# zezax/one

Hardware: AMD Instinct MI355X
Metric: GB/s input scanned (and Minput/s) for fixed DFA (higher is better)
Workload: dtype u8; 1 GPU; configs[1]: syn256 DFA (256 states used / 256 classes, REDA fmtDirect4), 1048576 lines x 64 B per GPU, match<styLast,false> -> result+start+end; input=uniformly random bytes, lines_per_gpu=1048576, line_len=64, rotating_input_buffers=6, working_set_bytes=402653184, streams=1, steps_per_call=32

## Files before the change

### one_amd/csrc/k_diag.h

```cpp
#pragma once

__global__ void __launch_bounds__(512)
k_diag_read(const uint4 *__restrict__ p, uint64_t n16, uint32_t *sink) {
  typedef uint32_t v4 __attribute__((ext_vector_type(4)));
  const v4 *q = reinterpret_cast<const v4 *>(p);
  const uint64_t step = uint64_t(gridDim.x) * 512;
  uint64_t i = uint64_t(blockIdx.x) * 512 + threadIdx.x;
  v4 acc = {0, 0, 0, 0};
  for (; i + 7 * step < n16; i += 8 * step) {
    v4 v[8];
#pragma unroll
    for (int k = 0; k < 8; ++k) v[k] = __builtin_nontemporal_load(q + i + k * step);
#pragma unroll
    for (int k = 0; k < 8; ++k) acc ^= v[k];
  }
  for (; i < n16; i += step) acc ^= q[i];
  uint32_t a = acc.x ^ acc.y ^ acc.z ^ acc.w;
  for (int o = 32; o; o >>= 1) a ^= __shfl_xor(a, o);
  if ((threadIdx.x & 63) == 0 && a == 0x9e3779b9u) atomicAdd(sink, 1u);
}

__global__ void __launch_bounds__(512)
k_diag_lines(const uint8_t *__restrict__ data, uint64_t nLines, int32_t *res, uint64_t *st,
             uint64_t *en, uint32_t *sink) {
  typedef uint32_t v4 __attribute__((ext_vector_type(4)));
  const uint64_t tiles = nLines / 1024;
  const uint64_t G = gridDim.x;
  if (blockIdx.x >= tiles) return;
  const uint64_t Q = (tiles - blockIdx.x + G - 1) / G;
  uint64_t ldT = blockIdx.x, ldQ = 0, t = blockIdx.x;
  v4 acc = {0, 0, 0, 0};
  v4 A[2][4], B[2][4];
  auto issue = [&](v4 (&blk)[2][4]) {
#pragma unroll
    for (int k = 0; k < 4; ++k)
#pragma unroll
      for (int c = 0; c < 2; ++c) {
        const uint64_t ln = ldT * 1024 + uint64_t(c) * 512 + threadIdx.x;
        blk[c][k] = reinterpret_cast<const v4 *>(data + ln * 64)[k];
      }
    if (ldQ + 1 < Q) { ++ldQ; ldT += G; }
  };
  auto walk = [&](const v4 (&blk)[2][4]) {
#pragma unroll
    for (int c = 0; c < 2; ++c) {
      const uint64_t ln = t * 1024 + uint64_t(c) * 512 + threadIdx.x;
      const v4 x = blk[c][0] ^ blk[c][1] ^ blk[c][2] ^ blk[c][3];
      acc ^= x;
      __builtin_nontemporal_store(int32_t(x.x), res + ln);
      __builtin_nontemporal_store(uint64_t(x.z), en + ln);
      __builtin_nontemporal_store(uint64_t(x.y), st + ln);
    }
    t += G;
  };
  issue(A);
  issue(B);
  walk(A);
  issue(A);
  for (uint64_t q = 1; q < Q; q += 2) {
    walk(B);
    if (q + 1 >= Q) break;
    issue(B);
    walk(A);
    issue(A);
  }
  if ((acc.x ^ acc.y ^ acc.z ^ acc.w) == 0x9e3779b9u) atomicAdd(sink, 1u);
}

__global__ void __launch_bounds__(512)
k_diag_long(const uint8_t *__restrict__ data, uint64_t nLines, uint32_t lineBytes, uint32_t *sink) {
  typedef uint32_t v4 __attribute__((ext_vector_type(4)));
  const uint64_t tiles = nLines / 1024;
  const uint32_t R = lineBytes / 128;
  v4 acc = {0, 0, 0, 0};
  for (uint64_t t = blockIdx.x; t < tiles; t += gridDim.x) {
    for (uint32_t r = 0; r < R; ++r) {
      v4 v[2][8];
#pragma unroll
      for (int k = 0; k < 8; ++k)
#pragma unroll
        for (int c = 0; c < 2; ++c) {
          const uint64_t ln = t * 1024 + uint64_t(c) * 512 + threadIdx.x;
          v[c][k] = reinterpret_cast<const v4 *>(data + ln * lineBytes + uint64_t(r) * 128)[k];
        }
#pragma unroll
      for (int c = 0; c < 2; ++c)
#pragma unroll
        for (int k = 0; k < 8; ++k) acc ^= v[c][k];
    }
  }
  if ((acc.x ^ acc.y ^ acc.z ^ acc.w) == 0x9e3779b9u) atomicAdd(sink, 1u);
}

template <int CH>
__global__ void __launch_bounds__(256)
k_diag_l2(const uint16_t *__restrict__ tab, uint32_t rounds, uint32_t *sink) {
  uint32_t idx[CH];
#pragma unroll
  for (int c = 0; c < CH; ++c)
    idx[c] = (blockIdx.x * 256u + threadIdx.x) * 2654435761u + uint32_t(c) * 40503u;
  for (uint32_t r = 0; r < rounds; ++r) {
#pragma unroll
    for (int c = 0; c < CH; ++c) {
      const uint32_t v = tab[idx[c] & 0xfffffu];
      idx[c] = idx[c] * 33u + v + r;
    }
  }
  uint32_t a = 0;
#pragma unroll
  for (int c = 0; c < CH; ++c) a ^= idx[c];
  if (a == 0x9e3779b9u) atomicAdd(sink, 1u);
}
```

### one_amd/csrc/k_stream_multi.h

```cpp
#pragma once

constexpr int kMultiMax = 32;

struct MultiPtrs {
  const uint8_t *data;
  int32_t *result;
  uint64_t *start;
  uint64_t *end;
  uint64_t n;
};

struct MultiIo {
  uint32_t nb;
  uint32_t lineLen;
  uint32_t tileStart[kMultiMax + 1];
  uint32_t ignoreAcceptUpTo;
  MultiPtrs b[kMultiMax];
};

typedef uint32_t u32x4_t __attribute__((ext_vector_type(4)));
__device__ __forceinline__ uint4 ntLoad16(const uint8_t *p) {
  const u32x4_t v = __builtin_nontemporal_load(reinterpret_cast<const u32x4_t *>(p));
  return make_uint4(v.x, v.y, v.z, v.w);
}

template <int MODE, int HALVES, int THREADS, int NT = 2, bool LEAN = false, int GR = 1,
          bool R1 = false>
__global__ void __launch_bounds__(THREADS)
k_stream_multi(DevDfa d, MultiIo m) {
  static_assert(MODE == kSmLastStartEnd || MODE == kSmLastEnd || MODE == kSmFullStart ||
                MODE == kSmFull, "the plain output modes only");
  static_assert(!LEAN || MODE != kSmFull, "styFull without start has no bookkeeping to defer");
  static_assert(GR == 1 || LEAN, "more than two chains per lane: the lean step only");
  static_assert(!R1 || (HALVES == 1 && !LEAN && GR == 1), "R1: the plain 64-byte walk only");
  constexpr uint32_t BLK = 64 * HALVES;
  constexpr int CH = kStreamChains * GR;
  constexpr bool kAcc = MODE == kSmLastStartEnd || MODE == kSmLastEnd;
  constexpr bool kStart = MODE == kSmLastStartEnd || MODE == kSmFullStart;
  constexpr uint32_t LPT = uint32_t(THREADS) * CH;
  __shared__ __align__(16) uint8_t lds[kStreamTabBytes + 1024];
  uint8_t *tab = lds;
  int32_t *ldsRes = reinterpret_cast<int32_t *>(lds + kStreamTabBytes);

  const uint32_t init = d.init, firstAccept = d.firstAccept;
  const uint32_t lineLen = m.lineLen;
  const uint32_t R = R1 ? 1u : lineLen / BLK;
  const uint32_t nTiles = m.tileStart[m.nb];
  const uint32_t G = gridDim.x;
  if (blockIdx.x >= nTiles) return;
  const uint32_t myTiles = (nTiles - blockIdx.x + G - 1) / G;
  const uint64_t Q = uint64_t(myTiles) * R;

  uint32_t ldTile = blockIdx.x, ldR = 0, ldK = 0;
  uint32_t ldLo = 0, ldHi = m.tileStart[1];
  const uint8_t *ldData = m.b[0].data;
  uint64_t ldN = m.b[0].n;
  uint64_t ldQ = 0;
  const uint8_t *ldP[CH];
  auto setLoadTile = [&]() {
    while (ldTile >= ldHi) {
      ++ldK;
      ldLo = ldHi;
      ldHi = m.tileStart[ldK + 1];
      ldData = m.b[ldK].data;
      ldN = m.b[ldK].n;
    }
    const uint64_t first = uint64_t(ldTile - ldLo) * LPT;
#pragma unroll
    for (int c = 0; c < CH; ++c) {
      uint64_t ln = first + uint64_t(c) * THREADS + threadIdx.x;
      if (ln >= ldN) ln = ldN - 1;
      ldP[c] = ldData + ln * lineLen;
    }
  };
  auto issue = [&](BlockRegs<HALVES> (&blk)[CH]) {
    const uint32_t byteOff = ldR * BLK;
#pragma unroll
    for (int k = 0; k < 4 * HALVES; ++k) {
#pragma unroll
      for (int c = 0; c < CH; ++c)
        blk[c].p[k] = (NT & 1)
                          ? ntLoad16(ldP[c] + byteOff + 16 * k)
                          : reinterpret_cast<const uint4 *>(ldP[c] + byteOff)[k];
    }
    if (ldQ + 1 < Q) {
      ++ldQ;
      if (++ldR == R) {
        ldR = 0;
        ldTile += G;
        setLoadTile();
      }
    }
  };

  const uint4 *tsrc = reinterpret_cast<const uint4 *>(d.table);
  const uint32_t n16 = d.tableBytes / 16;
  constexpr uint32_t kStagePieces = (kStreamTabBytes / 16 + THREADS - 1) / THREADS;
  uint4 tv[kStagePieces];
#pragma unroll
  for (uint32_t k = 0; k < kStagePieces; ++k) {
    const uint32_t i = k * THREADS + threadIdx.x;
    tv[k] = i < n16 ? tsrc[i] : make_uint4(0, 0, 0, 0);
  }
  const int32_t myRes = threadIdx.x < d.nStates ? d.result[threadIdx.x] : 0;
  BlockRegs<HALVES> A[CH], B[CH];
  setLoadTile();
  issue(A);
  {
    uint4 *dst = reinterpret_cast<uint4 *>(tab);
#pragma unroll
    for (uint32_t k = 0; k < kStagePieces; ++k) {
      const uint32_t i = k * THREADS + threadIdx.x;
      if (i < kStreamTabBytes / 16) dst[i] = tv[k];
    }
    if (threadIdx.x < 256) ldsRes[threadIdx.x] = myRes;
  }
  asm volatile("" : : "v"(tab) : "memory");
  __syncthreads();

  uint32_t tile = blockIdx.x, r = 0, wkK = 0;
  uint32_t wkLo = 0, wkHi = m.tileStart[1];
  int32_t *oRes = m.b[0].result;
  uint64_t *oStart = m.b[0].start, *oEnd = m.b[0].end;
  uint64_t oN = m.b[0].n;
  const uint8_t *oData = m.b[0].data;
  auto setWalkTile = [&]() {
    while (tile >= wkHi) {
      ++wkK;
      wkLo = wkHi;
      wkHi = m.tileStart[wkK + 1];
      oRes = m.b[wkK].result;
      oStart = m.b[wkK].start;
      oEnd = m.b[wkK].end;
      oN = m.b[wkK].n;
      if (LEAN) oData = m.b[wkK].data;
    }
  };
  setWalkTile();

  uint32_t s[CH], accS[CH], endv[CH], startv[CH];
  uint64_t mA[CH], mB[CH];
  LeanRegs L[GR];
  const uint32_t T8 = firstAccept << 8;

  auto walkLean = [&](const BlockRegs<HALVES> (&blk)[CH]) {
    if (r == 0) {
#pragma unroll
      for (int g = 0; g < GR; ++g) leanBegin(L[g], init);
    }
#pragma unroll
    for (int g = 0; g < GR; ++g) leanPin(L[g]);
    if (GR > 1) leanDrain();
#pragma unroll
    for (int h = 0; h < HALVES; ++h) {
#pragma unroll
      for (int q = 0; q < 4; ++q) {
        uint4 piece[CH];
#pragma unroll
        for (int c = 0; c < CH; ++c) piece[c] = blk[c].p[4 * h + q];
        leanWalk16<kAcc, kStart, GR>(piece, L, T8, init);
      }
    }
    if (GR > 1) leanDrain();
    if (r + 1 == R) {
      const uint32_t lane = threadIdx.x & 63;
      const uint64_t first = uint64_t(tile - wkLo) * LPT;
#pragma unroll
      for (int g = 0; g < GR; ++g) {
        LeanRegs &G = L[g];
        leanEnd(G, T8, init, kAcc, kStart);
        uint64_t ln[2];
        uint4 pa[2], ps[2];
        uint32_t PA[2], PS[2];
#pragma unroll
        for (int c = 0; c < 2; ++c) {
          ln[c] = first + uint64_t(2 * g + c) * THREADS + threadIdx.x;
          const uint64_t lc = ln[c] < oN ? ln[c] : oN - 1;
          const uint8_t *base = oData + lc * lineLen;
          PA[c] = G.recA[c] ? (G.recA[c] >> 8) - 1 : 0;
          PS[c] = G.recS[c] ? (G.recS[c] >> 8) - 1 : 0;
          if (kAcc) pa[c] = *reinterpret_cast<const uint4 *>(base + 16ull * PA[c]);
          if (kStart) ps[c] = *reinterpret_cast<const uint4 *>(base + 16ull * PS[c]);
        }
        int32_t rr[2];
        uint32_t en[2], sv[2];
        if (kAcc) {
          uint32_t s2[2];
          StreamBook b2[2];
          uint64_t u0[2] = {0, 0}, u1[2] = {0, 0};
#pragma unroll
          for (int c = 0; c < 2; ++c) { s2[c] = G.recA[c] & 0xffu; b2[c].acc = 0; b2[c].end = 0; b2[c].start = 0; }
          streamWalk16<kSmLastEnd, 0>(pa, s2, b2, u0, u1, firstAccept, init);
#pragma unroll
          for (int c = 0; c < 2; ++c) {
            uint32_t acc = b2[c].acc, er = b2[c].end;
            if (s2[c] >= firstAccept) { acc = s2[c]; er = 16; }
            const bool hit = G.recA[c] != 0;
            rr[c] = hit ? ldsRes[acc & 0xffu] : 0;
            en[c] = hit ? 16u * PA[c] + er : 0u;
          }
        } else {
#pragma unroll
          for (int c = 0; c < 2; ++c) {
            rr[c] = G.sX[c] >= firstAccept ? ldsRes[G.sX[c] & 0xffu] : 0;
            en[c] = lineLen;
          }
        }
        if (kStart) {
          uint32_t s3[2];
          StreamBook b3[2];
          uint64_t w0[2], w1[2];
#pragma unroll
          for (int c = 0; c < 2; ++c) {
            s3[c] = G.recS[c] & 0xffu;
            b3[c].acc = 0; b3[c].end = 0; b3[c].start = 0;
            w0[c] = __builtin_amdgcn_ballot_w64(s3[c] == init);
            w1[c] = w0[c];
          }
          streamWalk16<kSmFullStart, 0>(ps, s3, b3, w0, w1, firstAccept, init);
#pragma unroll
          for (int c = 0; c < 2; ++c) {
            uint32_t pos = b3[c].start ? b3[c].start - 1 : 0;
            if (((w0[c] >> lane) & 1) && s3[c] != init) pos = 15;
            sv[c] = G.recS[c] ? 16u * PS[c] + pos : 0u;
          }
        }
#pragma unroll
        for (int c = 0; c < 2; ++c) {
          if (ln[c] < oN) {
            __builtin_nontemporal_store(rr[c], oRes + ln[c]);
            if (oEnd) __builtin_nontemporal_store(rr[c] ? uint64_t(en[c]) : uint64_t(0), oEnd + ln[c]);
            if (kStart && oStart)
              __builtin_nontemporal_store(rr[c] ? uint64_t(sv[c]) : uint64_t(0), oStart + ln[c]);
          }
        }
      }
    }
    if (++r == R) {
      r = 0;
      tile += G;
      if (tile < nTiles) setWalkTile();
    }
  };

  auto walkBlock = [&](const BlockRegs<HALVES> (&blk)[CH]) {
    if constexpr (LEAN) {
      walkLean(blk);
    } else {
    if (r == 0) {
#pragma unroll
      for (int c = 0; c < CH; ++c) {
        s[c] = init; accS[c] = 0; endv[c] = 0; startv[c] = 0;
        mA[c] = ~0ull; mB[c] = ~0ull;
      }
    }
#pragma unroll
    for (int h = 0; h < HALVES; ++h) {
      StreamBook b[CH];
#pragma unroll
      for (int c = 0; c < CH; ++c) { b[c].acc = accS[c]; b[c].end = 0; b[c].start = 0; }
      uint4 piece[CH];
#pragma unroll
      for (int c = 0; c < CH; ++c) piece[c] = blk[c].p[4 * h + 0];
      streamWalk16<MODE, 0>(piece, s, b, mA, mB, firstAccept, init);
#pragma unroll
      for (int c = 0; c < CH; ++c) piece[c] = blk[c].p[4 * h + 1];
      streamWalk16<MODE, 1>(piece, s, b, mA, mB, firstAccept, init);
#pragma unroll
      for (int c = 0; c < CH; ++c) piece[c] = blk[c].p[4 * h + 2];
      streamWalk16<MODE, 2>(piece, s, b, mA, mB, firstAccept, init);
#pragma unroll
      for (int c = 0; c < CH; ++c) piece[c] = blk[c].p[4 * h + 3];
      streamWalk16<MODE, 3>(piece, s, b, mA, mB, firstAccept, init);
      const uint32_t off = r * BLK + h * 64;
#pragma unroll
      for (int c = 0; c < CH; ++c) {
        if (kAcc) {
          accS[c] = b[c].acc;
          endv[c] = b[c].end ? off + b[c].end : endv[c];
          if (s[c] >= firstAccept) { accS[c] = s[c]; endv[c] = off + 64; }
          if (endv[c] <= m.ignoreAcceptUpTo) { endv[c] = 0; accS[c] = 0; }
        }
        if (kStart) {
          startv[c] = b[c].start ? off + b[c].start - 1 : startv[c];
          const bool wasInit63 = (mA[c] >> (threadIdx.x & 63)) & 1;
          if (wasInit63 && s[c] != init) startv[c] = off + 63;
        }
      }
    }
    const bool lineEnd = r + 1 == R;
    const uint64_t first = uint64_t(tile - wkLo) * LPT;
#pragma unroll
    for (int c = 0; c < CH; ++c) {
      const uint64_t ln = first + uint64_t(c) * THREADS + threadIdx.x;
      const bool report = lineEnd && ln < oN;
      int32_t rr;
      uint32_t en;
      if (kAcc) {
        rr = ldsRes[accS[c] & 0xffu];
        rr = endv[c] ? rr : 0;
        en = endv[c];
      } else {
        rr = ldsRes[s[c] & 0xffu];
        rr = s[c] >= firstAccept ? rr : 0;
        en = lineLen;
      }
      int32_t *pr = report ? oRes + ln : reinterpret_cast<int32_t *>(d.sink);
      uint64_t *pe = report && oEnd ? oEnd + ln : reinterpret_cast<uint64_t *>(d.sink);
      uint64_t *ps = report && oStart ? oStart + ln : reinterpret_cast<uint64_t *>(d.sink);
      if ((NT & 2) && R == 1) {
        __builtin_nontemporal_store(rr, pr);
        __builtin_nontemporal_store(rr ? uint64_t(en) : uint64_t(0), pe);
        if (kStart) __builtin_nontemporal_store(rr ? uint64_t(startv[c]) : uint64_t(0), ps);
      } else {
        *pr = rr;
        *pe = rr ? uint64_t(en) : 0;
        if (kStart) *ps = rr ? uint64_t(startv[c]) : 0;
      }
    }
    if (++r == R) {
      r = 0;
      tile += G;
      if (tile < nTiles) setWalkTile();
    }
    }
  };

  issue(B);
  walkBlock(A);
  issue(A);
  for (uint64_t q = 1; q < Q; q += 2) {
    walkBlock(B);
    if (q + 1 >= Q) break;
    issue(B);
    walkBlock(A);
    issue(A);
  }
}

inline int multiLabInt(const char *name, int lo, int hi, int dflt) {
  const char *e = getenv(name);
  const int v = e ? atoi(e) : dflt;
  return v < lo || v > hi ? dflt : v;
}

template <int MODE, int NT, bool LEAN>
hipError_t launchStreamMultiN(const DevDfa &d, const MultiIo &m, const LaunchCfg &cfg,
                              hipStream_t stream) {
  static const int wgs = multiLabInt("REDGPU_MULTI_WGS", 1, 2, 2);
  const uint32_t tiles = m.tileStart[m.nb];
  const bool wide = m.lineLen % 128 == 0;
  const uint32_t want = uint32_t(cfg.numCUs) * uint32_t(wide ? 1 : wgs);
  const uint32_t blocks = tiles < want ? tiles : want;
  if constexpr (!LEAN) {
    if (m.lineLen == 64) {
      hipLaunchKernelGGL((k_stream_multi<MODE, 1, kStreamThreads, NT, false, 1, true>), dim3(blocks),
                         dim3(kStreamThreads), 0, stream, d, m);
      return hipGetLastError();
    }
  }
  if (wide)
    hipLaunchKernelGGL((k_stream_multi<MODE, 2, kStreamThreads, NT, LEAN>), dim3(blocks),
                       dim3(kStreamThreads), 0, stream, d, m);
  else
    hipLaunchKernelGGL((k_stream_multi<MODE, 1, kStreamThreads, NT, LEAN>), dim3(blocks),
                       dim3(kStreamThreads), 0, stream, d, m);
  return hipGetLastError();
}

template <int MODE>
hipError_t launchStreamLean4(const DevDfa &d, const MultiIo &m, const LaunchCfg &cfg,
                             hipStream_t stream) {
  MultiIo m4 = m;
  const uint64_t lpt = uint64_t(kStreamThreads) * kStreamChains * 2;
  for (uint32_t k = 0; k < m.nb; ++k)
    m4.tileStart[k + 1] = m4.tileStart[k] + uint32_t((m.b[k].n + lpt - 1) / lpt);
  for (uint32_t k = m.nb; k < uint32_t(kMultiMax); ++k) m4.tileStart[k + 1] = m4.tileStart[m.nb];
  const uint32_t tiles = m4.tileStart[m4.nb];
  const uint32_t blocks = tiles < uint32_t(cfg.numCUs) ? tiles : uint32_t(cfg.numCUs);
  hipLaunchKernelGGL((k_stream_multi<MODE, 1, kStreamThreads, 2, true, 2>), dim3(blocks),
                     dim3(kStreamThreads), 0, stream, d, m4);
  return hipGetLastError();
}

inline bool leanWanted(const MultiIo &m, const LaunchCfg &cfg) {
  static const int lab = multiLabInt("REDGPU_LEAN", 0, 1, 0);
  return (lab || cfg.forceLean) && m.lineLen >= kLeanMinLine && m.lineLen < (1u << 27);
}

template <int MODE>
hipError_t launchStreamMultiT(const DevDfa &d, const MultiIo &m, const LaunchCfg &cfg,
                              hipStream_t stream) {
  if constexpr (MODE != kSmFull) {
    if (leanWanted(m, cfg)) {
      if (cfg.leanChains4) return launchStreamLean4<MODE>(d, m, cfg, stream);
      return launchStreamMultiN<MODE, 2, true>(d, m, cfg, stream);
    }
  }
  if constexpr (MODE == kSmLastStartEnd) {
    static const int nt = multiLabInt("REDGPU_MULTI_NT", 0, 3, 2);
    if (nt == 0) return launchStreamMultiN<MODE, 0, false>(d, m, cfg, stream);
    if (nt == 1) return launchStreamMultiN<MODE, 1, false>(d, m, cfg, stream);
    if (nt == 3) return launchStreamMultiN<MODE, 3, false>(d, m, cfg, stream);
  }
  return launchStreamMultiN<MODE, 2, false>(d, m, cfg, stream);
}
```

### one_amd/csrc/kernels.hip

```cpp
#include "kernels.h"

#include <cstdlib>
#include <type_traits>

#include "../../include/redgpu.h"

#ifndef REDGPU_TU
#define REDGPU_TU 0
#endif
#define REDGPU_TU_STREAM (REDGPU_TU == 0 || REDGPU_TU == 1)
#define REDGPU_TU_RAGGED (REDGPU_TU == 0 || REDGPU_TU == 2)
#define REDGPU_TU_GENERIC (REDGPU_TU == 0 || REDGPU_TU == 3)
#define REDGPU_TU_GREP (REDGPU_TU == 0 || REDGPU_TU == 4)
#define REDGPU_TU_COLLECT_TEXT (REDGPU_TU == 0 || REDGPU_TU == 5)
#define REDGPU_TU_REPLACE_TEXT (REDGPU_TU == 0 || REDGPU_TU == 6)
#define REDGPU_TU_TALLY_TEXT (REDGPU_TU == 0 || REDGPU_TU == 7)

#define REDGPU_KIND_SWITCH(CALL)                                                          \
  switch (d.tableKind) {                                                                  \
  case REDGPU_TAB_LDS_FUSED_U8: return CALL(REDGPU_TAB_LDS_FUSED_U8);                     \
  case REDGPU_TAB_LDS_FUSED_U16: return CALL(REDGPU_TAB_LDS_FUSED_U16);                   \
  case REDGPU_TAB_LDS_CLASS_U16: return CALL(REDGPU_TAB_LDS_CLASS_U16);                   \
  case REDGPU_TAB_GLOBAL_U16: return CALL(REDGPU_TAB_GLOBAL_U16);                         \
  case REDGPU_TAB_HOT_ROWS: return CALL(REDGPU_TAB_HOT_ROWS);                               \
// ... 546 lines not shown
    return e;
  }
  *kernelName = "k_match_all_long";
  const uint64_t c = collectLongChunk(n, chunkBytes, cfg);
  MlBufs b{};
  b.m = (n + c - 1) / c;
  b.chunk = uint32_t(c);
  const uint64_t nb = (b.m + 1023) / 1024;
  auto up16 = [](uint64_t x) { return (x + 15) & ~uint64_t(15); };
  const size_t bytes = up16(b.m * 8) * 2 + up16(nb * 8) * 2 + up16(b.m * 4) * 5 + 64;
  void *scratch = nullptr;
  hipError_t e = raggedScratch(stream, bytes, &scratch);
  if (e != hipSuccess) return e;
  uint8_t *q = static_cast<uint8_t *>(scratch);
  b.esc = reinterpret_cast<uint64_t *>(q); q += up16(b.m * 8);
  b.off = reinterpret_cast<uint64_t *>(q); q += up16(b.m * 8);
  b.blockOff = reinterpret_cast<uint64_t *>(q); q += up16(nb * 8);
  b.blockEsc = reinterpret_cast<uint64_t *>(q); q += up16(nb * 8);
  b.ent = reinterpret_cast<uint32_t *>(q); q += up16(b.m * 4);
  b.exit = reinterpret_cast<uint32_t *>(q); q += up16(b.m * 4);
  b.cnt = reinterpret_cast<uint32_t *>(q); q += up16(b.m * 4);
  b.head = reinterpret_cast<uint32_t *>(q); q += up16(b.m * 4);
  b.work = reinterpret_cast<uint32_t *>(q); q += up16(b.m * 4);
  b.ctl = reinterpret_cast<uint32_t *>(q);
  *ctl = b.ctl;
  const int lead = doLeader && d.leaderLen > 0 ? 1 : 0;
#define ML_CALL(K) launchMatchAllLongK<K>(d, data, n, b, lead, cap, count, result, start, end, cfg, stream)
  REDGPU_KIND_SWITCH(ML_CALL)
#undef ML_CALL
}

template <int KIND>
hipError_t launchReplaceK(const DevDfa &d, const Batch &b, int style, int lead, const uint8_t *repl,
                          uint64_t replLen, uint64_t max, uint64_t *counts, uint64_t *outLens,
                          const uint64_t *outOffsets, uint8_t *out, uint64_t outCap,
                          const LaunchCfg &cfg, hipStream_t stream) {
  constexpr bool kLds = Tab<KIND>::kInLds || KIND == REDGPU_TAB_HOT_ROWS;
  constexpr int kThreads = kLds ? 1024 : 256;
  const size_t ldsBytes = 512 + ldsTableBytes<KIND>(d);
  hipError_t e = setLds(k_replace<KIND, kThreads>, ldsBytes);
  if (e != hipSuccess) return e;
  uint64_t blocks = (b.n + kThreads - 1) / kThreads;
  const uint64_t perCu = kLds ? (ldsBytes <= 80 * 1024 ? 2 : 1) : 8;
  const uint64_t capBlocks = uint64_t(cfg.numCUs) * perCu;
  if (blocks > capBlocks) blocks = capBlocks;
  if (blocks == 0) blocks = 1;
  hipLaunchKernelGGL((k_replace<KIND, kThreads>), dim3(uint32_t(blocks)), dim3(kThreads), ldsBytes,
                     stream, d, b, style, lead, repl, replLen, max, counts, outLens, outOffsets,
                     out, outCap);
  return hipGetLastError();
}

static hipError_t launchReplacePass(const DevDfa &d, const Batch &b, int style, int lead,
                                    const uint8_t *repl, uint64_t replLen, uint64_t max,
                                    uint64_t *counts, uint64_t *outLens,
                                    const uint64_t *outOffsets, uint8_t *out, uint64_t outCap,
                                    const LaunchCfg &cfg, hipStream_t stream) {
#define RP_CALL(K) launchReplaceK<K>(d, b, style, lead, repl, replLen, max, counts, outLens, \
                                     outOffsets, out, outCap, cfg, stream)
  REDGPU_KIND_SWITCH(RP_CALL)
#undef RP_CALL
}

hipError_t launchReplace(const DevDfa &d, const Batch &b, int style, int doLeader,
                         const uint8_t *repl, uint64_t replLen, uint64_t max, uint64_t *counts,
                         uint64_t *outOffsets, uint8_t *out, uint64_t outCap,
                         const LaunchCfg &cfg, hipStream_t stream) {
  if (b.n == 0) return hipSuccess;
  const int lead = doLeader && d.leaderLen > 0;
  const uint64_t nPart = (b.n + 1023) / 1024;
  void *scratch = nullptr;
  hipError_t e = raggedScratch(stream, size_t(b.n + nPart) * 8 + 64, &scratch);
  if (e != hipSuccess) return e;
  uint64_t *lens = static_cast<uint64_t *>(scratch);
  uint64_t *partials = lens + b.n;
  e = launchReplacePass(d, b, style, lead, repl, replLen, max, counts, lens, nullptr, nullptr, 0,
                        cfg, stream);
  if (e != hipSuccess) return e;
  hipLaunchKernelGGL(k_scan_partials, dim3(uint32_t(nPart)), dim3(256), 0, stream, lens, b.n,
                     partials);
  hipLaunchKernelGGL(k_scan_tops, dim3(1), dim3(1024), 0, stream, partials, nPart);
  hipLaunchKernelGGL(k_scan_fill, dim3(uint32_t(nPart)), dim3(256), 0, stream, lens, b.n, partials,
                     outOffsets);
  e = hipGetLastError();
  if (e != hipSuccess || !out) return e;
  return launchReplacePass(d, b, style, lead, repl, replLen, max, counts, lens, outOffsets, out,
                           outCap, cfg, stream);
}

uint64_t splitChunks(uint64_t len) { return (len + kSplitChunk - 1) / kSplitChunk; }

uint64_t splitMaskBytes(uint64_t len) { return splitChunks(len) * (kSplitChunk / 8); }

static uint32_t splitGroups(uint64_t nChunks) {
  return uint32_t((nChunks + kSplitGroup - 1) / kSplitGroup);
}

hipError_t launchSplitLines(const uint8_t *data, uint64_t len, uint8_t delim, uint64_t *offsets,
                            uint64_t cap, uint64_t *nLines, uint32_t *counts, uint64_t *bases,
                            uint16_t *masks, hipStream_t stream) {
  const uint64_t nChunks = splitChunks(len);
  const uint32_t groups = splitGroups(nChunks);
  if (nChunks)
    hipLaunchKernelGGL(k_split_count, dim3(groups), dim3(kSplitThreads), 0, stream, data, len,
                       uint32_t(delim), nChunks, counts, masks);
  hipLaunchKernelGGL(k_split_scan, dim3(1), dim3(1024), 0, stream, counts, nChunks, bases, nLines,
                     offsets, cap);
  if (nChunks)
    hipLaunchKernelGGL(k_split_scatter, dim3(groups), dim3(kSplitThreads), 0, stream, masks,
                       nChunks, bases, offsets, cap);
  return hipGetLastError();
}

hipError_t launchTextIndex(const uint8_t *data, uint64_t len, uint8_t delim, uint64_t *nLines,
                           uint32_t *counts, uint64_t *bases, uint16_t *masks, uint64_t *open,
                           uint16_t *zeroMasks, uint64_t *spare, int numCUs, hipStream_t stream) {
  const uint64_t nChunks = splitChunks(len);
  if (nChunks) {
    hipLaunchKernelGGL(k_split_count, dim3(splitGroups(nChunks)), dim3(kSplitThreads), 0, stream,
                       data, len, uint32_t(delim), nChunks, counts, masks);
  }
  hipLaunchKernelGGL(k_split_scan, dim3(1), dim3(1024), 0, stream, counts, nChunks, bases,
                     nLines ? nLines : spare, spare + 1, uint64_t(0));
  if (nChunks) {
    uint64_t small = (nChunks + 3) / 4;
    if (small > uint64_t(numCUs) * 8) small = uint64_t(numCUs) * 8;
    hipLaunchKernelGGL(k_gp_last, dim3(uint32_t(small)), dim3(256), 0, stream, masks, counts,
                       nChunks, open, zeroMasks);
    hipLaunchKernelGGL(k_gp_open, dim3(1), dim3(1024), 0, stream, open, nChunks);
  }
  return hipGetLastError();
}

hipError_t launchDiagRead(const void *data, uint64_t bytes, uint32_t *sink, int numCUs,
                          hipStream_t stream) {
  if (bytes < 16) return hipSuccess;
  hipLaunchKernelGGL(k_diag_read, dim3(uint32_t(numCUs)), dim3(512), 0, stream,
                     static_cast<const uint4 *>(data), bytes / 16, sink);
  return hipGetLastError();
}

hipError_t launchDiagL2(const uint16_t *table, uint32_t rounds, uint32_t *sink, int numCUs,
                        hipStream_t stream, uint64_t *lookups) {
  constexpr int kCh = 2;
  hipLaunchKernelGGL((k_diag_l2<kCh>), dim3(uint32_t(numCUs) * 8), dim3(256), 0, stream, table, rounds,
                     sink);
  if (lookups) *lookups = uint64_t(numCUs) * 8 * 256 * kCh * rounds;
  return hipGetLastError();
}

hipError_t launchDiagLines(const uint8_t *data, uint64_t nLines, uint32_t lineBytes, int32_t *res,
                           uint64_t *st, uint64_t *en, uint32_t *sink, int numCUs,
                           hipStream_t stream) {
  if (nLines < 1024) return hipSuccess;
  if (lineBytes != 64) {
    hipLaunchKernelGGL(k_diag_long, dim3(uint32_t(numCUs)), dim3(512), 0, stream, data, nLines,
                       lineBytes, sink);
    return hipGetLastError();
  }
  const uint64_t tiles = nLines / 1024, want = uint64_t(numCUs) * 2;
  hipLaunchKernelGGL(k_diag_lines, dim3(uint32_t(tiles < want ? tiles : want)), dim3(512), 0,
                     stream, data, nLines, res, st, en, sink);
  return hipGetLastError();
}

template <int KIND>
hipError_t launchWalkedK(const DevDfa &d, const Batch &b, int lead, unsigned long long *walked,
                         const LaunchCfg &cfg, hipStream_t stream) {
  constexpr bool kLds = Tab<KIND>::kInLds || KIND == REDGPU_TAB_HOT_ROWS;
  constexpr int kThreads = kLds ? 1024 : 256;
  const size_t ldsBytes = 512 + ldsTableBytes<KIND>(d);
  hipError_t e = setLds(k_walked<KIND, kThreads>, ldsBytes);
  if (e != hipSuccess) return e;
  uint64_t blocks = (b.n + kThreads - 1) / kThreads;
  const uint64_t perCu = kLds ? (ldsBytes <= 80 * 1024 ? 2 : 1) : 8;
  const uint64_t capBlocks = uint64_t(cfg.numCUs) * perCu;
  if (blocks > capBlocks) blocks = capBlocks;
  if (blocks == 0) blocks = 1;
  hipLaunchKernelGGL((k_walked<KIND, kThreads>), dim3(uint32_t(blocks)), dim3(kThreads), ldsBytes,
                     stream, d, b, lead, walked);
  return hipGetLastError();
}

hipError_t launchWalked(const DevDfa &d, const Batch &b, int doLeader, unsigned long long *walked,
                        const LaunchCfg &cfg, hipStream_t stream) {
  if (b.n == 0) return hipSuccess;
  const int lead = doLeader && d.leaderLen > 0;
#define WK_CALL(K) launchWalkedK<K>(d, b, lead, walked, cfg, stream)
  REDGPU_KIND_SWITCH(WK_CALL)
#undef WK_CALL
}

hipError_t launchVisits(const DevDfa &d, const Batch &b, uint32_t *hist, const LaunchCfg &cfg,
                        hipStream_t stream) {
  if (b.n == 0) return hipSuccess;
#define VI_CALL(K) launchVisitsK<K>(d, b, hist, cfg, stream)
  REDGPU_KIND_SWITCH(VI_CALL)
#undef VI_CALL
}

hipError_t launchAdvance(const DevDfa &d, const Batch &b, uint32_t *state, const LaunchCfg &cfg,
                         hipStream_t stream, const char **kernelName) {
  *kernelName = "k_advance";
  if (b.n == 0) return hipSuccess;
  bool handled = false;
  hipError_t se = launchAdvanceStream(d, b, state, cfg, stream, kernelName, &handled);
  if (handled || se != hipSuccess) return se;
#define AD_CALL(K) launchAdvanceK<K>(d, b, state, cfg, stream)
  REDGPU_KIND_SWITCH(AD_CALL)
#undef AD_CALL
}

#endif

[[maybe_unused]] static void normalizeVerbStyle(const DevDfa &d, const LaunchCfg &cfg, bool lead, int &verb,
                               int &style) {
  if (d.suffixClosed && !lead) {
    if (verb == kScan) verb = kCheck;
    else if (verb == kSearch) verb = kMatch;
  }
  if (verb == kCheck && !lead && d.uniformResult && !d.earlyDeath && !cfg.forceGeneric &&
      (style == kStyInstant || style == kStyFirst || style == kStyTangent))
    style = kStyLast;
}

#if REDGPU_TU_GREP || REDGPU_TU_COLLECT_TEXT
struct RecordScratch {
  uint64_t *bases, *open, *recBases;
  uint32_t *counts, *recCounts;
  uint64_t *misc;
  uint16_t *masks, *hitMasks;
  uint64_t bytes;
  RecordScratch(void *scratch, uint64_t nChunks) {
    Carve c{static_cast<uint8_t *>(scratch)};
    bases = c.take<uint64_t>(nChunks);
    open = c.take<uint64_t>(nChunks);
    recBases = c.take<uint64_t>(nChunks);
    counts = c.take<uint32_t>(nChunks);
    recCounts = c.take<uint32_t>(nChunks);
    misc = c.take<uint64_t>(4);
    c.align(16);
    masks = c.take<uint16_t>(nChunks * (kSplitChunk / 16));
    hitMasks = c.take<uint16_t>(nChunks * (kSplitChunk / 16));
    bytes = c.at;
  }
};
#endif

#if REDGPU_TU_GREP
uint64_t grepScratchBytes(uint64_t len) { return RecordScratch(nullptr, splitChunks(len)).bytes; }

hipError_t launchGrepText(const DevDfa &d, int style, int doLeader, int invert, const uint8_t *data,
                          uint64_t len, uint8_t delim, uint64_t maxCount, uint64_t cap,
                          uint64_t *nLines, uint64_t *nSelected, uint64_t *line, uint64_t *begin,
                          uint64_t *finish, int32_t *result, uint64_t *start, uint64_t *end,
                          void *scratch, const LaunchCfg &cfg, hipStream_t stream,
                          const char **kernelName) {
  *kernelName = "k_grep_text";
  const uint64_t nChunks = splitChunks(len);
  const RecordScratch m(scratch, nChunks);
  uint64_t *dummy = m.misc + 1, *total = m.misc + 2;
  const hipError_t e = launchTextIndex(data, len, delim, nLines, m.counts, m.bases, m.masks, m.open,
                                       m.hitMasks, m.misc, cfg.numCUs, stream);
  if (e != hipSuccess) return e;
  const int lead = doLeader && d.leaderLen > 0 ? 1 : 0;
  int verb = kSearch;
  normalizeVerbStyle(d, cfg, lead != 0, verb, style);
  const GpBufs b{m.masks, m.hitMasks, m.bases, m.open, m.recCounts, m.recBases, nChunks};
  const GpOut out{cap < maxCount ? cap : maxCount, line, begin, finish, result, start, end};
  const bool write = out.limit > 0 && (line || begin || finish || result || start || end);
#define GP_ARGS d, data, b, style, lead, invert, out, write, total, maxCount, nSelected, m.recBases, \
                dummy, cfg, stream
#define GP_CALL(K) \
  (verb == kSearch ? launchGrepK<K, kSearch>(GP_ARGS) : launchGrepK<K, kMatch>(GP_ARGS))
  REDGPU_KIND_SWITCH(GP_CALL)
#undef GP_CALL
#undef GP_ARGS
}
#endif

#if REDGPU_TU_COLLECT_TEXT
uint64_t collectTextScratchBytes(uint64_t len) {
  return RecordScratch(nullptr, splitChunks(len)).bytes;
}

hipError_t launchCollectText(const DevDfa &d, const uint8_t *data, uint64_t len, uint8_t delim,
                             uint64_t cap, uint64_t *nLines, uint64_t *nMatches, uint64_t *line,
                             uint64_t *begin, int32_t *result, uint64_t *start, uint64_t *end,
                             void *scratch, const LaunchCfg &cfg, hipStream_t stream,
                             const char **kernelName) {
  *kernelName = "k_collect_text";
  const uint64_t nChunks = splitChunks(len);
  const RecordScratch m(scratch, nChunks);
  uint64_t *dummy = m.misc + 1;
  const hipError_t e = launchTextIndex(data, len, delim, nLines, m.counts, m.bases, m.masks, m.open,
                                       m.hitMasks, m.misc, cfg.numCUs, stream);
  if (e != hipSuccess) return e;
  const GpBufs b{m.masks, m.hitMasks, m.bases, m.open, m.recCounts, m.recBases, nChunks};
  const CtOut out{cap, line, begin, result, start, end};
  const bool write = cap > 0 && (line || begin || result || start || end);
#define CT_CALL(K) \
  launchCollectTextK<K>(d, data, b, out, write, nMatches, m.recBases, dummy, cfg, stream)
  REDGPU_KIND_SWITCH(CT_CALL)
#undef CT_CALL
}
#endif

#if REDGPU_TU_TALLY_TEXT
struct TallyScratch {
  uint64_t *bases, *open;
  uint64_t *misc;
  uint16_t *masks;
  uint32_t *counts;
  uint64_t bytes;
  TallyScratch(void *scratch, uint64_t nChunks) {
// ... 235 lines not shown
```

Before: 4203 GB/s.

## Add dedicated 1024-thread single-buffer kernel for 64-byte lines

Replaces the 64-byte-line path of the streaming multi-batch kernel with a new k_stream_multi_r1 kernel. It uses 1024 threads per block and a waves-per-EU hint, and keeps a single register buffer. The loads for the next tile are issued right after the DFA walk of the current tile and before its result stores, so memory latency is hidden by occupancy instead of by double-buffering. Tiles are recomputed for the larger block size, and the diagnostic lines kernel is reworked the same way. This lowers register pressure and raises resident waves, at the cost of less per-thread prefetch depth and fewer, larger tiles per CU.

```diff
diff --git a/one_amd/csrc/k_diag.h b/one_amd/csrc/k_diag.h
--- a/one_amd/csrc/k_diag.h
+++ b/one_amd/csrc/k_diag.h
@@ -20,50 +20,51 @@
   if ((threadIdx.x & 63) == 0 && a == 0x9e3779b9u) atomicAdd(sink, 1u);
 }
 
-__global__ void __launch_bounds__(512)
+template <int THREADS>
+__global__ void __launch_bounds__(THREADS)
 k_diag_lines(const uint8_t *__restrict__ data, uint64_t nLines, int32_t *res, uint64_t *st,
              uint64_t *en, uint32_t *sink) {
   typedef uint32_t v4 __attribute__((ext_vector_type(4)));
-  const uint64_t tiles = nLines / 1024;
+  constexpr uint64_t LPT = 2 * uint64_t(THREADS);
+  const uint64_t tiles = nLines / LPT;
   const uint64_t G = gridDim.x;
   if (blockIdx.x >= tiles) return;
   const uint64_t Q = (tiles - blockIdx.x + G - 1) / G;
-  uint64_t ldT = blockIdx.x, ldQ = 0, t = blockIdx.x;
+  uint64_t ldT = blockIdx.x, ldQ = 0;
   v4 acc = {0, 0, 0, 0};
-  v4 A[2][4], B[2][4];
-  auto issue = [&](v4 (&blk)[2][4]) {
-#pragma unroll
-    for (int k = 0; k < 4; ++k)
-#pragma unroll
-      for (int c = 0; c < 2; ++c) {
-        const uint64_t ln = ldT * 1024 + uint64_t(c) * 512 + threadIdx.x;
-        blk[c][k] = reinterpret_cast<const v4 *>(data + ln * 64)[k];
-      }
-    if (ldQ + 1 < Q) { ++ldQ; ldT += G; }
-  };
-  auto walk = [&](const v4 (&blk)[2][4]) {
+  v4 X[4][2];
+  auto request = [&](int k) {
 #pragma unroll
     for (int c = 0; c < 2; ++c) {
-      const uint64_t ln = t * 1024 + uint64_t(c) * 512 + threadIdx.x;
-      const v4 x = blk[c][0] ^ blk[c][1] ^ blk[c][2] ^ blk[c][3];
-      acc ^= x;
-      __builtin_nontemporal_store(int32_t(x.x), res + ln);
-      __builtin_nontemporal_store(uint64_t(x.z), en + ln);
-      __builtin_nontemporal_store(uint64_t(x.y), st + ln);
+      const uint64_t ln = ldT * LPT + uint64_t(c) * THREADS + threadIdx.x;
+      X[k][c] = reinterpret_cast<const v4 *>(data + ln * 64)[k];
     }
-    t += G;
   };
-  issue(A);
-  issue(B);
-  walk(A);
-  issue(A);
-  for (uint64_t q = 1; q < Q; q += 2) {
-    walk(B);
-    if (q + 1 >= Q) break;
-    issue(B);
-    walk(A);
-    issue(A);
-  }
+  auto walk = [&]() {
+    const uint64_t t = ldT;
+    v4 x[2];
+#pragma unroll
+    for (int k = 0; k < 4; ++k) {
+#pragma unroll
+      for (int c = 0; c < 2; ++c) x[c] = k ? x[c] ^ X[k][c] : X[k][c];
+    }
+    if (ldQ + 1 < Q) { ++ldQ; ldT += G; }
+#pragma unroll
+    for (int k = 0; k < 4; ++k) request(k);
+    __builtin_amdgcn_sched_barrier(0);
+#pragma unroll
+    for (int c = 0; c < 2; ++c) {
+      const uint64_t ln = t * LPT + uint64_t(c) * THREADS + threadIdx.x;
+      acc ^= x[c];
+      __builtin_nontemporal_store(int32_t(x[c].x), res + ln);
+      __builtin_nontemporal_store(uint64_t(x[c].z), en + ln);
+      __builtin_nontemporal_store(uint64_t(x[c].y), st + ln);
+    }
+  };
+#pragma unroll
+  for (int k = 0; k < 4; ++k) request(k);
+  walk();
+  for (uint64_t q = 1; q < Q; ++q) walk();
   if ((acc.x ^ acc.y ^ acc.z ^ acc.w) == 0x9e3779b9u) atomicAdd(sink, 1u);
 }
 
diff --git a/one_amd/csrc/k_stream_multi.h b/one_amd/csrc/k_stream_multi.h
--- a/one_amd/csrc/k_stream_multi.h
+++ b/one_amd/csrc/k_stream_multi.h
@@ -24,15 +24,13 @@
   return make_uint4(v.x, v.y, v.z, v.w);
 }
 
-template <int MODE, int HALVES, int THREADS, int NT = 2, bool LEAN = false, int GR = 1,
-          bool R1 = false>
+template <int MODE, int HALVES, int THREADS, int NT = 2, bool LEAN = false, int GR = 1>
 __global__ void __launch_bounds__(THREADS)
 k_stream_multi(DevDfa d, MultiIo m) {
   static_assert(MODE == kSmLastStartEnd || MODE == kSmLastEnd || MODE == kSmFullStart ||
                 MODE == kSmFull, "the plain output modes only");
   static_assert(!LEAN || MODE != kSmFull, "styFull without start has no bookkeeping to defer");
   static_assert(GR == 1 || LEAN, "more than two chains per lane: the lean step only");
-  static_assert(!R1 || (HALVES == 1 && !LEAN && GR == 1), "R1: the plain 64-byte walk only");
   constexpr uint32_t BLK = 64 * HALVES;
   constexpr int CH = kStreamChains * GR;
   constexpr bool kAcc = MODE == kSmLastStartEnd || MODE == kSmLastEnd;
@@ -44,7 +42,7 @@
 
   const uint32_t init = d.init, firstAccept = d.firstAccept;
   const uint32_t lineLen = m.lineLen;
-  const uint32_t R = R1 ? 1u : lineLen / BLK;
+  const uint32_t R = lineLen / BLK;
   const uint32_t nTiles = m.tileStart[m.nb];
   const uint32_t G = gridDim.x;
   if (blockIdx.x >= nTiles) return;
@@ -338,6 +336,153 @@
   }
 }
 
+constexpr int kResidentThreads = 1024;
+
+template <int MODE, int THREADS, int NT = 2>
+__global__ void __launch_bounds__(THREADS) __attribute__((amdgpu_waves_per_eu(THREADS / 128)))
+k_stream_multi_r1(DevDfa d, MultiIo m) {
+  static_assert(MODE == kSmLastStartEnd || MODE == kSmLastEnd || MODE == kSmFullStart ||
+                MODE == kSmFull, "the plain output modes only");
+  constexpr int CH = kStreamChains;
+  constexpr bool kAcc = MODE == kSmLastStartEnd || MODE == kSmLastEnd;
+  constexpr bool kStart = MODE == kSmLastStartEnd || MODE == kSmFullStart;
+  constexpr uint32_t LPT = uint32_t(THREADS) * CH;
+  __shared__ __align__(16) uint8_t lds[kStreamTabBytes + 1024];
+  uint8_t *tab = lds;
+  int32_t *ldsRes = reinterpret_cast<int32_t *>(lds + kStreamTabBytes);
+
+  const uint32_t init = d.init, firstAccept = d.firstAccept;
+  const uint32_t nTiles = m.tileStart[m.nb];
+  const uint32_t G = gridDim.x;
+  if (blockIdx.x >= nTiles) return;
+  const uint32_t Q = (nTiles - blockIdx.x + G - 1) / G;
+
+  uint32_t ldTile = blockIdx.x, ldK = 0, ldQ = 0;
+  uint32_t ldLo = 0, ldHi = m.tileStart[1];
+  MultiPtrs ldB = m.b[0];
+  uint64_t ldFirst = 0;
+  uint32_t ldLast = 0;
+  auto setLoadTile = [&]() {
+    while (ldTile >= ldHi) {
+      ++ldK;
+      ldLo = ldHi;
+      ldHi = m.tileStart[ldK + 1];
+      ldB = m.b[ldK];
+    }
+    ldFirst = uint64_t(ldTile - ldLo) * LPT;
+    const uint64_t left = ldB.n - ldFirst;
+    ldLast = left < LPT ? uint32_t(left) - 1u : LPT - 1u;
+  };
+  uint4 X[4][CH];
+  auto request = [&](int k) {
+    const uint8_t *base = ldB.data + ldFirst * 64u + 16u * uint32_t(k);
+#pragma unroll
+    for (int c = 0; c < CH; ++c) {
+      const uint32_t l = uint32_t(c) * THREADS + threadIdx.x;
+      const uint32_t off = (l < ldLast ? l : ldLast) * 64u;
+      X[k][c] = (NT & 1) ? ntLoad16(base + off) : *reinterpret_cast<const uint4 *>(base + off);
+    }
+  };
+
+  const uint4 *tsrc = reinterpret_cast<const uint4 *>(d.table);
+  const uint32_t n16 = d.tableBytes / 16;
+  constexpr uint32_t kStagePieces = (kStreamTabBytes / 16 + THREADS - 1) / THREADS;
+  uint4 tv[kStagePieces];
+#pragma unroll
+  for (uint32_t k = 0; k < kStagePieces; ++k) {
+    const uint32_t i = k * THREADS + threadIdx.x;
+    tv[k] = i < n16 ? tsrc[i] : make_uint4(0, 0, 0, 0);
+  }
+  const int32_t myRes = threadIdx.x < d.nStates ? d.result[threadIdx.x] : 0;
+  setLoadTile();
+#pragma unroll
+  for (int k = 0; k < 4; ++k) request(k);
+  {
+    uint4 *dst = reinterpret_cast<uint4 *>(tab);
+#pragma unroll
+    for (uint32_t k = 0; k < kStagePieces; ++k) {
+      const uint32_t i = k * THREADS + threadIdx.x;
+      if (i < kStreamTabBytes / 16) dst[i] = tv[k];
+    }
+    if (threadIdx.x < 256) ldsRes[threadIdx.x] = myRes;
+  }
+  asm volatile("" : : "v"(tab) : "memory");
+  __syncthreads();
+
+  auto walkTile = [&]() {
+    const uint32_t wkLast = ldLast;
+    int32_t *const oRes = ldB.result + ldFirst;
+    uint64_t *const oEnd = ldB.end ? ldB.end + ldFirst : nullptr;
+    uint64_t *const oStart = ldB.start ? ldB.start + ldFirst : nullptr;
+    uint32_t s[CH];
+    uint64_t mA[CH], mB[CH];
+    StreamBook b[CH];
+#pragma unroll
+    for (int c = 0; c < CH; ++c) {
+      s[c] = init; mA[c] = ~0ull; mB[c] = ~0ull;
+      b[c].acc = 0; b[c].end = 0; b[c].start = 0;
+    }
+    streamWalk16<MODE, 0>(X[0], s, b, mA, mB, firstAccept, init);
+    streamWalk16<MODE, 1>(X[1], s, b, mA, mB, firstAccept, init);
+    streamWalk16<MODE, 2>(X[2], s, b, mA, mB, firstAccept, init);
+    streamWalk16<MODE, 3>(X[3], s, b, mA, mB, firstAccept, init);
+    if (ldQ + 1 < Q) {
+      ++ldQ;
+      ldTile += G;
+      setLoadTile();
+    }
+#pragma unroll
+    for (int k = 0; k < 4; ++k) request(k);
+#pragma unroll
+    for (int c = 0; c < CH; ++c) {
+      int32_t rr;
+      uint32_t en, sv = 0;
+      if (kAcc) {
+        uint32_t acc = b[c].acc;
+        en = b[c].end;
+        if (s[c] >= firstAccept) { acc = s[c]; en = 64; }
+        if (en <= m.ignoreAcceptUpTo) { en = 0; acc = 0; }
+        rr = ldsRes[acc & 0xffu];
+        rr = en ? rr : 0;
+      } else {
+        rr = ldsRes[s[c] & 0xffu];
+        rr = s[c] >= firstAccept ? rr : 0;
+        en = 64;
+      }
+      if (kStart) {
+        sv = b[c].start ? b[c].start - 1 : 0;
+        const bool wasInit63 = (mA[c] >> (threadIdx.x & 63)) & 1;
+        if (wasInit63 && s[c] != init) sv = 63;
+      }
+      const uint32_t l = uint32_t(c) * THREADS + threadIdx.x;
+      const uint32_t ln = l < wkLast ? l : wkLast;
+      int32_t *pr = oRes + ln;
+      uint64_t *pe = oEnd ? oEnd + ln : reinterpret_cast<uint64_t *>(d.sink);
+      uint64_t *ps = oStart ? oStart + ln : reinterpret_cast<uint64_t *>(d.sink);
+      if (NT & 2) {
+        __builtin_nontemporal_store(rr, pr);
+        __builtin_nontemporal_store(rr ? uint64_t(en) : uint64_t(0), pe);
+        if (kStart) __builtin_nontemporal_store(rr ? uint64_t(sv) : uint64_t(0), ps);
+      } else {
+        *pr = rr;
+        *pe = rr ? uint64_t(en) : 0;
+        if (kStart) *ps = rr ? uint64_t(sv) : 0;
+      }
+    }
+  };
+
+  walkTile();
+  for (uint32_t q = 1; q < Q; ++q) walkTile();
+}
+
+inline MultiIo retiled(const MultiIo &m, uint64_t lpt) {
+  MultiIo r = m;
+  for (uint32_t k = 0; k < m.nb; ++k)
+    r.tileStart[k + 1] = r.tileStart[k] + uint32_t((m.b[k].n + lpt - 1) / lpt);
+  for (uint32_t k = m.nb; k < uint32_t(kMultiMax); ++k) r.tileStart[k + 1] = r.tileStart[m.nb];
+  return r;
+}
+
 inline int multiLabInt(const char *name, int lo, int hi, int dflt) {
   const char *e = getenv(name);
   const int v = e ? atoi(e) : dflt;
@@ -354,8 +499,11 @@
   const uint32_t blocks = tiles < want ? tiles : want;
   if constexpr (!LEAN) {
     if (m.lineLen == 64) {
-      hipLaunchKernelGGL((k_stream_multi<MODE, 1, kStreamThreads, NT, false, 1, true>), dim3(blocks),
-                         dim3(kStreamThreads), 0, stream, d, m);
+      const MultiIo mr = retiled(m, uint64_t(kResidentThreads) * kStreamChains);
+      const uint32_t rtiles = mr.tileStart[mr.nb];
+      hipLaunchKernelGGL((k_stream_multi_r1<MODE, kResidentThreads, NT>),
+                         dim3(rtiles < want ? rtiles : want), dim3(kResidentThreads), 0, stream, d,
+                         mr);
       return hipGetLastError();
     }
   }
@@ -371,11 +519,7 @@
 template <int MODE>
 hipError_t launchStreamLean4(const DevDfa &d, const MultiIo &m, const LaunchCfg &cfg,
                              hipStream_t stream) {
-  MultiIo m4 = m;
-  const uint64_t lpt = uint64_t(kStreamThreads) * kStreamChains * 2;
-  for (uint32_t k = 0; k < m.nb; ++k)
-    m4.tileStart[k + 1] = m4.tileStart[k] + uint32_t((m.b[k].n + lpt - 1) / lpt);
-  for (uint32_t k = m.nb; k < uint32_t(kMultiMax); ++k) m4.tileStart[k + 1] = m4.tileStart[m.nb];
+  const MultiIo m4 = retiled(m, uint64_t(kStreamThreads) * kStreamChains * 2);
   const uint32_t tiles = m4.tileStart[m4.nb];
   const uint32_t blocks = tiles < uint32_t(cfg.numCUs) ? tiles : uint32_t(cfg.numCUs);
   hipLaunchKernelGGL((k_stream_multi<MODE, 1, kStreamThreads, 2, true, 2>), dim3(blocks),
diff --git a/one_amd/csrc/kernels.hip b/one_amd/csrc/kernels.hip
--- a/one_amd/csrc/kernels.hip
+++ b/one_amd/csrc/kernels.hip
@@ -722,15 +722,16 @@
 hipError_t launchDiagLines(const uint8_t *data, uint64_t nLines, uint32_t lineBytes, int32_t *res,
                            uint64_t *st, uint64_t *en, uint32_t *sink, int numCUs,
                            hipStream_t stream) {
-  if (nLines < 1024) return hipSuccess;
   if (lineBytes != 64) {
+    if (nLines < 1024) return hipSuccess;
     hipLaunchKernelGGL(k_diag_long, dim3(uint32_t(numCUs)), dim3(512), 0, stream, data, nLines,
                        lineBytes, sink);
     return hipGetLastError();
   }
-  const uint64_t tiles = nLines / 1024, want = uint64_t(numCUs) * 2;
-  hipLaunchKernelGGL(k_diag_lines, dim3(uint32_t(tiles < want ? tiles : want)), dim3(512), 0,
-                     stream, data, nLines, res, st, en, sink);
+  const uint64_t tiles = nLines / (2 * uint64_t(kResidentThreads)), want = uint64_t(numCUs) * 2;
+  if (tiles == 0) return hipSuccess;
+  hipLaunchKernelGGL(k_diag_lines<kResidentThreads>, dim3(uint32_t(tiles < want ? tiles : want)),
+                     dim3(kResidentThreads), 0, stream, data, nLines, res, st, en, sink);
   return hipGetLastError();
 }
 
```

After: 4621 GB/s, median of 6. 9.9% higher.
